# QData/ChromeGCN

Hardware: AMD Instinct MI355X
Metric: GCN windows/sec (2-layer, d_model=128) on GM12878 Hi-C graph (higher is better)
Workload: dtype f32

## Files before the change

chromegcn_amd/csrc/cgcn_common.hpp:

```cpp
#pragma once
#include <hip/hip_runtime.h>
#include <stdint.h>

#include "chromegcn.h"

typedef float f32x4 __attribute__((ext_vector_type(4)));
typedef float f32x2 __attribute__((ext_vector_type(2)));

#define WAVE 64
#define TILE_NODES 16
#ifndef BWD_MAX_PARTIALS
#define BWD_MAX_PARTIALS 256
#endif

typedef __bf16 bf16x8 __attribute__((ext_vector_type(8)));
typedef __bf16 bf16x2 __attribute__((ext_vector_type(2)));
typedef uint32_t u32x4 __attribute__((ext_vector_type(4)));
typedef uint32_t u32x2 __attribute__((ext_vector_type(2)));
__device__ __forceinline__ uint32_t sp_pack(float x0, float x1) {
  return __builtin_bit_cast(uint32_t, __builtin_convertvector((f32x2){x0, x1}, bf16x2));
}
__device__ __forceinline__ float sp_lo(uint32_t pk) { return __uint_as_float(pk << 16); }
__device__ __forceinline__ float sp_up(uint32_t pk) { return __uint_as_float(pk & 0xffff0000u); }
__device__ __forceinline__ void sp_split2(float x0, float x1, uint32_t& h, uint32_t& m, uint32_t& l) {
// ... 182 lines not shown
__device__ __forceinline__ void bacc_add(unsigned long long* b, int S, int D, int slot, int s, int c, double sdy, double sdyx,
                                         int fa, int fb) {
  unsigned long long* w = b + ((size_t)(slot * S + s) * D + c) * 2;
  const double va = ldexp(sdy, fa), vb = ldexp(sdyx, fb);
  if (!(__builtin_fabs(va) < 1.15e18) || !(__builtin_fabs(vb) < 1.15e18)) {
    atomicOr(b + (size_t)STAT_ACC_SLOTS * S * D * 2 + BACC_FLAG, 1ull);
    atomicOr(b + (size_t)STAT_ACC_SLOTS * S * D * 2 + BACC_LOSS, BACC_LOSS_BAD);
    return;
  }
  atomicAdd(&w[0], (unsigned long long)(long long)__builtin_rint(va));
  atomicAdd(&w[1], (unsigned long long)(long long)__builtin_rint(vb));
}
__device__ __forceinline__ void bacc_get(const unsigned long long* __restrict__ b, int S, int D, int s, int c, int n, float& c0, float& c1) {
  long long ta = 0, tb = 0;
#pragma unroll
  for (int slot = 0; slot < STAT_ACC_SLOTS; ++slot) {
    const unsigned long long* w = b + ((size_t)(slot * S + s) * D + c) * 2;
    ta += (long long)w[0];
    tb += (long long)w[1];
  }
  const unsigned long long* h = b + (size_t)STAT_ACC_SLOTS * S * D * 2;
  const int fa = (int)(unsigned)(h[BACC_EXP] & 0xFFFFFFFFull) - 1024, fb = (int)(unsigned)(h[BACC_EXP] >> 32) - 1024;
  const double invn = 1.0 / (double)n;
  c0 = (float)(ldexp((double)ta, -fa) * invn);
  c1 = (float)(ldexp((double)tb, -fb) * invn);
  if (h[BACC_FLAG] != 0ull) c0 = c1 = __builtin_nanf("");
}
__device__ __forceinline__ void stat_acc_add(unsigned long long* acc, int S, int D, int slot, int s, int c, double sum1, double sum2,
                                             double lim = 4194304.0) {
  const double sc = (double)(1ll << STAT_ACC_FBITS);
  unsigned long long* w = acc + ((size_t)(slot * S + s) * D + c) * 2;
  if (!(__builtin_fabs(sum1) < lim) || !(sum2 < lim)) {
    atomicOr(acc + (size_t)STAT_ACC_SLOTS * S * D * 2, 1ull);
    return;
  }
  atomicAdd(&w[0], (unsigned long long)(long long)__builtin_rint(sum1 * sc));
  atomicAdd(&w[1], (unsigned long long)(long long)__builtin_rint(sum2 * sc));
}
__device__ __forceinline__ void stat_acc_get(const unsigned long long* __restrict__ acc, int S, int D, int s, int c, int n,
                                             double& mean, double& m2) {
  long long t1 = 0, t2 = 0;
#pragma unroll
  for (int slot = 0; slot < STAT_ACC_SLOTS; ++slot) {
    const unsigned long long* w = acc + ((size_t)(slot * S + s) * D + c) * 2;
    t1 += (long long)w[0];
    t2 += (long long)w[1];
  }
  const double isc = 1.0 / (double)(1ll << STAT_ACC_FBITS);
  const double s1 = (double)t1 * isc, s2 = (double)t2 * isc;
  mean = s1 / (double)n;
  m2 = s2 - mean * s1;
  if (m2 < 0.0) m2 = 0.0;
  if (acc[(size_t)STAT_ACC_SLOTS * S * D * 2] != 0ull) mean = m2 = __builtin_nan("");
}

#define HEAD_STREAM_ID 0x4845u

struct HeadApply {
  const float* dym;
  const float* bnc;
  const unsigned long long* bacc;
  const float* mean;
  const float* invstd;
  const float* bn_w;
  const unsigned long long* rng_state;
  float keep_scale;
  uint32_t thresh;
  int S;
  const float* hf_part;
  float* hf_dWout;
  float* hf_dbout;
  int hf_P, hf_C, hf_CP, hf_accumulate;
  const float* dloss;
  float* hf_dbn_w;
  float* hf_dbn_b;
};

__host__ __device__ __forceinline__ constexpr int head_part_stride(int CP, int D) { return CP * D + CP + 8 * D; }
#define HEAD_STAT_COLS 16

template <int NT, bool EXT = false>
__device__ __forceinline__ void head_finalize_slab(int slab, int P, int D, int C, int CP,
                                                   const float* __restrict__ part, float* __restrict__ dWout,
                                                   float* __restrict__ dbout, int accumulate,
                                                   const float* __restrict__ dloss, void* scratch = nullptr) {
  constexpr int NS = NT / 64;
  const float gl = dloss ? dloss[0] : 1.f;
  const int PS = head_part_stride(CP, D);
  const int total = CP * D + CP;
  float (*hred)[64];
  if constexpr (EXT) {
    hred = (float (*)[64])scratch;
  } else {
    __shared__ __attribute__((aligned(16))) float hred_own[NS][64];
    hred = hred_own;
  }
  const int lane = threadIdx.x & 63, wave = threadIdx.x >> 6;
  const int el4 = lane & 15, sub = lane >> 4;
  const int e0 = slab * 64 + el4 * 4;
  f32x4 a = {0.f, 0.f, 0.f, 0.f};
  if (e0 < total) {
    const int per = (P + NS * 4 - 1) / (NS * 4);
    const int p0 = (wave * 4 + sub) * per, p1 = min(P, p0 + per);
    for (int p = p0; p < p1; p += 8) {
      f32x4 t[8];
#pragma unroll
// ... 117 lines not shown
```

chromegcn_amd/csrc/cgcn_head.hip:

```cpp
#include "cgcn_common.hpp"

#define HEAD_STAT_BLOCKS 128
#define HEAD_TILE 16
#define HEADB_TILE 32
#ifndef HEAD_MAX_PARTIALS
#define HEAD_MAX_PARTIALS 256
#endif


template <int D>
__global__ __launch_bounds__(256) void k_head_colstats(int n, int S, int rows_per_blk, const float* __restrict__ X,
                                                       float* __restrict__ part) {
  constexpr int RL = 256 / D;
  __shared__ float sm[2][256];
  const int c = threadIdx.x % D, rl = threadIdx.x / D;
  const int r0 = blockIdx.x * rows_per_blk, r1 = min(n, r0 + rows_per_blk);
  for (int s = 0; s < S; ++s) {
    const float* Xs = X + (size_t)s * n * D + c;
    const float pivot = r0 < n ? fmaxf(Xs[(size_t)r0 * D], 0.f) : 0.f;
    float s1 = 0.f, s2 = 0.f;
    int i = r0 + rl;
    for (; i + 3 * RL < r1; i += 4 * RL) {
      float v[4];
#pragma unroll
// ... 976 lines not shown
      for (int e = 0; e < EPL; ++e) {
        const int c = lane * EPL + e;
        const float g = gv[e];
#pragma unroll
        for (int s = 0; s < 2; ++s) {
          if (s < S) {
            float dy = g * invS;
            if (thresh) dy = dropout_keep(key, (uint32_t)(((size_t)s * n + i) * D + c), thresh) ? dy * keep_scale : 0.f;
            const float xh = (fmaxf(xv[t][s][e], 0.f) - mu[s][e]) * is[s][e];
            sdy[s][e] += dy;
            sdyx[s][e] += dy * xh;
          }
        }
      }
    }
    __syncthreads();
  }

  HF_STAMP(10);
  float* P = part + (size_t)blockIdx.x * PS;
#pragma unroll
  for (int ib = 0; ib < CBMAX; ++ib)
#pragma unroll
    for (int jb = 0; jb < JBW; ++jb)
#pragma unroll
      for (int e = 0; e < 4; ++e)
        if (c0 + ib * 16 < CPT) P[(size_t)(c0 + ib * 16 + q * 4 + e) * D + (wave * JBW + jb) * 16 + r] = accW[ib][jb][e];
  if (threadIdx.x < CP && c0 + (int)threadIdx.x < CPT) P[CPT * D + c0 + threadIdx.x] = dbo;
  HF_STAMP(11);
  lacc = wave_sum(lacc);
  if (lane == 0) lsum[wave] = lacc;
  if (last) {
    unsigned long long* bb = sa.acc ? bacc_base(sa.acc, S, D) : nullptr;
    int fa = 0, fb = 0;
    if (sa.acc) {
      head_bacc_points(wmax, NW, keep_scale, n, fa, fb);
      if (blockIdx.x == 0 && threadIdx.x == 0)
        bb[(size_t)STAT_ACC_SLOTS * S * D * 2 + BACC_EXP] = ((unsigned long long)(unsigned)(fb + 1024) << 32) | (unsigned long long)(unsigned)(fa + 1024);
    }
    head_stats_partial<D, NW, TR * LDY>(Yt, (double*)(P + CPT * D + CPT), sdy, sdyx, wave, lane, bb, S, fa, fb);
  }
  __syncthreads();
  if (threadIdx.x == 0) {
    float t = 0.f;
#pragma unroll
    for (int w = 0; w < NW; ++w) t += lsum[w];
    const float tl = first ? t : loss_part[blockIdx.x] + t;
    loss_part[blockIdx.x] = tl;
    if (sa.acc && last) head_loss_ticket(sa, S, D, tl, inv_count);
  }
  HF_STAMP(12);
}

#if (defined(HRSX_NOBACC) || defined(HRSX_NOSTAGE) || defined(HRSX_NOTICKET)) && !defined(CGCN_EXPERIMENT_BUILD)
#error "HRSX_* are decomposition switches (garbage results): build a variant with -DCGCN_EXPERIMENT_BUILD (tools/mkvariant.py), never the shipped library"
#endif
#ifndef HEAD_RS
#define HEAD_RS 1
#endif
#ifndef HEAD_NT_PROBS
#define HEAD_NT_PROBS 0
#endif
#ifndef HEAD_RS_PRIO
#define HEAD_RS_PRIO 0
#endif
#ifdef RS_TIMING
__device__ unsigned long long rs_stamps[8 * 2 * 8];
#ifndef RS_STAMP_K
#define RS_STAMP_K 1
#endif
#define RS_STAMP(i)                                                                                        \
  do {                                                                                                     \
    __builtin_amdgcn_s_waitcnt(0);                                                                         \
    if (k == RS_STAMP_K && (threadIdx.x == 0 || threadIdx.x == 512) && (blockIdx.x & 31) == 0)             \
      rs_stamps[((blockIdx.x >> 5) * 2 + (threadIdx.x >> 9)) * 8 + (i)] = wall_clock64();                  \
  } while (0)
extern "C" int cgcn_debug_rs_stamps(unsigned long long* out) {
  return hipMemcpyFromSymbol(out, HIP_SYMBOL(rs_stamps), sizeof(unsigned long long) * 8 * 2 * 8) == hipSuccess ? 0 : -1;
}
#else
#define RS_STAMP(i)
#endif
template <bool MULTI, int NB, bool DROP, int NRB = 2>
__global__ __launch_bounds__(1024) void k_head_fused_rs(int n, int S, int C, const float* __restrict__ X,
                                                        const float* __restrict__ bn_w, const float* __restrict__ bn_b,
                                                        const float* __restrict__ mean, const float* __restrict__ invstd,
                                                        const float* __restrict__ Wout, const float* __restrict__ bout,
                                                        const float* __restrict__ target, float keep_scale, uint32_t thresh,
                                                        const unsigned long long* __restrict__ rng_state, float inv_count,
                                                        float* __restrict__ probs, float* __restrict__ loss_part,
                                                        float* __restrict__ dym, float* __restrict__ part,
                                                        int c0, int Cp, int CPT, int first_, int last_, HeadStatAcc sa) {
  constexpr int D = 128, TR = 16 * NRB, EPL = 2, RPW = TR / 8, KQ = D / 4;
  constexpr int CP = 128, CBMAX = 8;
  constexpr int LDP = CP + 18, LDY = D + 16, LDW = D + 16;
  __shared__ __attribute__((aligned(16))) float Wl[NB * 16 * LDW];
  __shared__ __attribute__((aligned(16))) float Pt[2][TR * LDP];
  __shared__ __attribute__((aligned(16))) float Yt[2][TR * LDY];
  __shared__ float lsum[8];
  __shared__ float wmax[16];
  const bool first = MULTI ? first_ != 0 : true, last = MULTI ? last_ != 0 : true;

  const int lane = threadIdx.x & 63;
  const int wave = __builtin_amdgcn_readfirstlane(threadIdx.x >> 6);
  const int own = wave & 7;
  const uint32_t key = DROP ? dropout_key(rng_state, HEAD_STREAM_ID) : 0u;
  const float invS = 1.f / (float)S;
// ... 642 lines not shown
        const int c = own * 16 + r;
#pragma unroll
        for (int e = 0; e < 4; ++e) {
          const int i = node0 + q * 4 + e;
          const float g = accY[e];
          if (i < n) dym[(unsigned)(i * D + c)] = g;
          if (last) {
#pragma unroll
            for (int s = 0; s < 2; ++s) {
              float dy = g * invS;
              if (DROP) dy = dropout_keep(key, (uint32_t)((s * n + i) * D + c), thresh) ? dy * keep_scale : 0.f;
              if (s == 1) dy = S2 ? dy : 0.f;
              const float xh = (fmaxf(xq[s][e], 0.f) - mu[s]) * is[s];
              sdy[s] += dy;
              sdyx[s] += dy * xh;
            }
          }
        }
      }
      __syncthreads();
      if (k < mt) load_xq((int)blockIdx.x + k * G);
      if (k >= 1) {
        int lq = lane;
        asm volatile("" : "+v"(lq));
        const int hh = lq >> 5, c16 = (lq >> 4) & 1, qp = (lq & 15) >> 2, pp = lq & 3;
        const int cbk = own >> 1, lb0 = 2 * (own & 1);
        const unsigned char* __restrict__ Pb = Ptb[(k - 1) & 1];
        const unsigned char* __restrict__ Yb = Ytb[(k - 1) & 1];
        int ty[2], tp[2];
#pragma unroll
        for (int rd = 0; rd < 2; ++rd) {
          const int row = 8 * hh + 4 * rd + qp, sg = sp_sigma(row);
          ty[rd] = row * 256 + (((4 * cbk + 2 * c16 + (pp >> 1)) ^ sg) << 4) + ((pp & 1) << 3);
          tp[rd] = row * 256 + (((4 * lb0 + 2 * c16 + (pp >> 1)) ^ sg) << 4) + ((pp & 1) << 3);
        }
        bf16x8 yf[3];
#pragma unroll
        for (int v = 0; v < 3; ++v) yf[v] = tr_pair(Yb + v * LVT + ty[0], Yb + v * LVT + ty[1]);
#pragma unroll
        for (int bb = 0; bb < 2; ++bb) {
          bf16x8 pf[3];
#pragma unroll
          for (int v = 0; v < 3; ++v) pf[v] = tr_pair(Pb + v * LVT + (tp[0] ^ (bb << 6)), Pb + v * LVT + (tp[1] ^ (bb << 6)));
          accW[bb] = __builtin_amdgcn_mfma_f32_32x32x16_bf16(pf[2], yf[0], accW[bb], 0, 0, 0);
          accW[bb] = __builtin_amdgcn_mfma_f32_32x32x16_bf16(pf[0], yf[2], accW[bb], 0, 0, 0);
          accW[bb] = __builtin_amdgcn_mfma_f32_32x32x16_bf16(pf[1], yf[1], accW[bb], 0, 0, 0);
          accW[bb] = __builtin_amdgcn_mfma_f32_32x32x16_bf16(pf[1], yf[0], accW[bb], 0, 0, 0);
          accW[bb] = __builtin_amdgcn_mfma_f32_32x32x16_bf16(pf[0], yf[1], accW[bb], 0, 0, 0);
          accW[bb] = __builtin_amdgcn_mfma_f32_32x32x16_bf16(pf[0], yf[0], accW[bb], 0, 0, 0);
        }
      }
      __syncthreads();
    }
    {
      const int hh = lane >> 5, cbk = own >> 1, lb0 = 2 * (own & 1);
#pragma unroll
      for (int bb = 0; bb < 2; ++bb)
#pragma unroll
        for (int e = 0; e < 16; ++e) {
          const int lab = 32 * (lb0 + bb) + (e & 3) + 8 * (e >> 2) + 4 * hh;
          if (c0 + (lab & ~15) < CPT) P[(size_t)(c0 + lab) * D + 32 * cbk + (lane & 31)] = accW[bb][e];
        }
    }
    const int r = lane & 15, q = lane >> 4;
    if (last) {
      double* out = (double*)(P + CPT * D + CPT);
#pragma unroll
      for (int s = 0; s < 2; ++s) {
        double a = (double)sdy[s], b = (double)sdyx[s];
        a += __shfl_xor(a, 16); a += __shfl_xor(a, 32);
        b += __shfl_xor(b, 16); b += __shfl_xor(b, 32);
        if (q == 0) {
          out[s * D + own * 16 + r] = a;
          out[(2 + s) * D + own * 16 + r] = b;
          if (sa.acc && s < S) {
            int fa, fb;
            head_bacc_points(wmax, 16, keep_scale, n, fa, fb);
            unsigned long long* bb = bacc_base(sa.acc, S, D);
#ifndef HRSX_NOBACC
            bacc_add(bb, S, D, (int)blockIdx.x & (STAT_ACC_SLOTS - 1), s, own * 16 + r, a, b, fa, fb);
#endif
            if (blockIdx.x == 0 && s == 0 && own == 0 && r == 0)
              bb[(size_t)STAT_ACC_SLOTS * S * D * 2 + BACC_EXP] = ((unsigned long long)(unsigned)(fb + 1024) << 32) | (unsigned long long)(unsigned)(fa + 1024);
          }
        }
      }
    }
    __syncthreads();
  }
#undef OPAQUE_LANE
}

__global__ __launch_bounds__(512) void k_head_bwd_finalize(int wslab0, int wslabs, int P, int n, int S, int D, int C, int CP,
                                                           const float* __restrict__ part, float* __restrict__ dWout,
                                                           float* __restrict__ dbout, float* __restrict__ dbn_w,
                                                           float* __restrict__ dbn_b, float* __restrict__ bnc,
                                                           int accumulate, const float* __restrict__ dloss) {
  if ((int)blockIdx.x < wslabs)
    head_finalize_slab<512>(wslab0 + blockIdx.x, P, D, C, CP, part, dWout, dbout, accumulate, dloss);
  else
    head_stats_finalize<512>((int)blockIdx.x - wslabs, P, n, S, D, CP, part, dbn_w, dbn_b, bnc, accumulate, dloss);
}

__global__ __launch_bounds__(512) void k_head_train_finish(int P, int n, int S, int D, int CP,
                                                           const float* __restrict__ part, float* __restrict__ bnc,
                                                           const float* __restrict__ loss_part, float inv_count,
// ... 360 lines not shown
```

chromegcn_amd/csrc/cgcn_kernels.hip:

```cpp
#include <atomic>
#include <type_traits>
#include <cstdlib>

#include "cgcn_common.hpp"

template <int S, int D>
struct Geo {
  static constexpr int PAY = S * D;
  static constexpr bool HALF = (PAY == 128);
  static constexpr int NV = HALF ? 1 : PAY / 256;
  static_assert(PAY == 128 || PAY == 256 || PAY == 512, "unsupported payload");
  __device__ static __forceinline__ int strand(int v, int lane) { return HALF ? 0 : ((v * 64 + lane) * 4) / D; }
  __device__ static __forceinline__ int column(int v, int lane) { return HALF ? (lane & 31) * 4 : ((v * 64 + lane) * 4) % D; }
};

#ifndef GU_OVERRIDE
#define GU_OVERRIDE 0
#endif
#ifndef NT_SAVED
#define NT_SAVED 0
#endif
#if NT_SAVED
#define NT_STORE4(p, v) __builtin_nontemporal_store((v), (f32x4*)(p))
#define NT_STORE1(p, v) __builtin_nontemporal_store((v), (p))
// ... 956 lines not shown
#pragma unroll
        for (int rr = 0; rr < R; ++rr) {
          v[rr] = St[(s * R + rr) * LD + c];
          sum += rr < cnt ? v[rr] : 0.f;
        }
        const float mean = sum * inv;
        float m2 = 0.f;
#pragma unroll
        for (int rr = 0; rr < R; ++rr) m2 += rr < cnt ? (v[rr] - mean) * (v[rr] - mean) : 0.f;
        chan_combine(st_cnt, st_mean, st_m2, (float)cnt, mean, m2);
      }
    }
  }
  if (colstats && threadIdx.x < S * D && tfirst < tend) {
    if (stat_acc) {
      const double nb = (double)st_cnt, mb = (double)st_mean;
      stat_acc_add((unsigned long long*)colstats, S, D, (int)blockIdx.x & (STAT_ACC_SLOTS - 1), (int)threadIdx.x / D,
                   (int)threadIdx.x % D, nb * mb, (double)st_m2 + nb * mb * mb);
    } else {
      float* out = colstats + ((size_t)blockIdx.x * S * D + threadIdx.x) * 2;
      out[0] = st_mean;
      out[1] = st_m2;
    }
  }
}

#ifndef RING_SLOTS
#define RING_SLOTS 8
#endif
#ifndef RING_ROW_WAVES
#define RING_ROW_WAVES 8
#endif
#define RING_THREADS ((RING_ROW_WAVES + 8) * 64)
#ifndef RING_PF
#define RING_PF 2
#endif
#ifndef RING_PF_HEAD
#define RING_PF_HEAD 2
#endif
#ifndef RING_PRIO
#define RING_PRIO 1
#endif
#ifndef RING_OPBUF
#define RING_OPBUF 2
#endif
#ifndef RING_EARLY_FLAG
#define RING_EARLY_FLAG 1
#endif
#ifndef RING_PRIME
#define RING_PRIME 0
#endif
#if (defined(RING_NO_WAIT) || defined(RING_SKIP_MFMA) || defined(RING_SKIP_ROWTEAM) || defined(RING_SKIP_LOADS) || \
     defined(RING_TEST_SLOW_ROW) || defined(RING_TEST_SLOW_MATRIX) || defined(RL256_SKIP_MFMA) || defined(RL256_SKIP_LOADS) || \
     defined(BSX_NORIDERS) || defined(BSX_NODXN) || defined(BSX_NOSTORE)) && \
    !defined(CGCN_EXPERIMENT_BUILD)
#error "RING_NO_WAIT / RING_SKIP_* / RING_TEST_SLOW_* are experiment switches: build a variant with -DCGCN_EXPERIMENT_BUILD (tools/mkvariant.py), never the shipped library"
#endif
#if defined(RING_TEST_SLOW_ROW) || defined(RING_TEST_SLOW_MATRIX)
__device__ __forceinline__ void ring_test_delay(int wave, int it) {
  unsigned h = (unsigned)wave * 2654435761u ^ (unsigned)it * 40503u ^ (unsigned)blockIdx.x * 97u;
  h ^= h >> 7;
  for (unsigned i = 0; i < (h & 15u); ++i) __builtin_amdgcn_s_sleep(10);
}
#endif
__device__ __forceinline__ void ring_wait(const unsigned* flag, unsigned target) {
#ifdef RING_NO_WAIT
  return;
#endif
  unsigned long long t0 = 0;
  for (unsigned spins = 1;; ++spins) {
    const unsigned v = __builtin_amdgcn_readfirstlane(__hip_atomic_load(flag, __ATOMIC_RELAXED, __HIP_MEMORY_SCOPE_WORKGROUP));
    if ((int)(v - target) >= 0) break;
    if ((spins & 0xFFFFu) == 0u) {
      const unsigned long long now = __builtin_amdgcn_s_memrealtime();
      if (t0 == 0) t0 = now;
      else if (now - t0 > 1000000000ull) __builtin_trap();
    }
    __builtin_amdgcn_s_sleep(1);
  }
  asm volatile("" ::: "memory");
}
__device__ __forceinline__ void ring_arrive(unsigned* flag, int lane) {
  asm volatile("s_waitcnt lgkmcnt(0)" ::: "memory");
  if (lane == 0) __hip_atomic_fetch_add(flag, 1u, __ATOMIC_RELAXED, __HIP_MEMORY_SCOPE_WORKGROUP);
}
#ifndef RING_SLOTS_SP
#define RING_SLOTS_SP 6
#endif
template <bool HEAD, bool DROP, int PROD>
__global__ __launch_bounds__(RING_THREADS) void k_bwd_rowlocal_ring(int M, int n, const float* __restrict__ dXn,
                                                            const float* __restrict__ Z, const float* __restrict__ X,
                                                            const float* __restrict__ gate, const float* __restrict__ dgate,
                                                            const float* __restrict__ H, const float* __restrict__ wg,
                                                            const float* __restrict__ rs, float* __restrict__ dHs,
                                                            float* __restrict__ part, HeadApply hp,
                                                            float* __restrict__ dxn_store, int row_blocks, int head_slabs,
                                                            const float* __restrict__ W) {
  constexpr int D = 128, SR = 16, NSL = PROD ? RING_SLOTS_SP : RING_SLOTS, PF = HEAD ? RING_PF_HEAD : RING_PF;
  constexpr int SLOT_F = PROD ? 3 * SR * D / 2 : SR * D;
  constexpr int LVB = SR * D * 2;
  constexpr int NRW = RING_ROW_WAVES;
  constexpr int NT = RING_THREADS;
  constexpr int RT = SR / (2 * NRW);
  static_assert(NRW * 2 * RT == SR && (NRW == 4 || NRW == 8), "row-team geometry");
  constexpr int PSTRIDE = D * D + 2 * D + 4;
  constexpr int RS = 2 * D + 4;
  __shared__ __attribute__((aligned(16))) float Hs[NSL][SLOT_F];
// ... 176 lines not shown
          unsigned char* hb = (unsigned char*)Hs[slot] + wo;
          *(u32x2*)hb = h2;
          *(u32x2*)(hb + LVB) = m2;
          *(u32x2*)(hb + 2 * LVB) = l2;
          sp_split4(du[t], h2, m2, l2);
          unsigned char* ub = (unsigned char*)Us[slot] + wo;
          *(u32x2*)ub = h2;
          *(u32x2*)(ub + LVB) = m2;
          *(u32x2*)(ub + 2 * LVB) = l2;
        } else {
          *(f32x4*)&Hs[slot][rowi * D + ((l ^ ((rowi & 1) << 2)) << 2)] = w.h[t];
          *(f32x4*)&Us[slot][rowi * D + ((l ^ rowi) << 2)] = du[t];
        }
        if (l == 0) Sc[slot][rowi] = w.sc[t];
      }
#endif
      ring_arrive(&FULL[slot], lane);
    };
#ifdef RING_SKIP_ROWTEAM
    __syncthreads();
    for (int it = 0; it < ns; ++it) {
      if (it >= NSL) ring_wait(&FREE[it % NSL], 8u * (unsigned)(it / NSL));
      ring_arrive(&FULL[it % NSL], lane);
    }
#else
#pragma unroll
    for (int j = 0; j < PF; ++j)
      if (j < ns) load_slot(j, R_[j]);
    __syncthreads();
    for (int it0 = 0; it0 < ns; it0 += PF) {
#pragma unroll
      for (int j = 0; j < PF; ++j) {
        const int it = it0 + j;
        if (it < ns) {
          row_pass(it, R_[j]);
          if (it + PF < ns) load_slot(it + PF, R_[j]);
        }
      }
    }
#endif
#pragma unroll
    for (int e = 0; e < 4; ++e) {
      db_acc[e] += __shfl_xor(db_acc[e], 32);
      dwg_acc[e] += __shfl_xor(dwg_acc[e], 32);
    }
    dcg_acc += __shfl_xor(dcg_acc, 32);
    if (!upper) {
      *(f32x4*)&red[wave][4 * l] = db_acc;
      *(f32x4*)&red[wave][D + 4 * l] = dwg_acc;
      if (l == 0) red[wave][2 * D] = dcg_acc;
    }
    ring_arrive(DONE, lane);
    ring_wait(DONE, (unsigned)NRW);
    for (int c = threadIdx.x; c < 2 * D + 1; c += NRW * 64) {
      float sacc = 0.f;
#pragma unroll
      for (int w = 0; w < NRW; ++w) sacc += red[w][c];
      P[D * D + c] = sacc;
    }
  } else if constexpr (PROD != 0) {
    const int own = wave - NRW;
    int lq = lane;
    asm volatile("" : "+v"(lq));
    const int r16 = lq & 15, q4 = lq >> 4;
    bf16x8 th[4], tm[4], tl[4];
#pragma unroll
    for (int s4 = 0; s4 < 4; ++s4) {
      float v[8];
      const f32x4 v0 = dHs ? *(const f32x4*)&W[(size_t)(16 * own + r16) * D + 32 * s4 + 8 * q4] : (f32x4){0.f, 0.f, 0.f, 0.f};
      const f32x4 v1 = dHs ? *(const f32x4*)&W[(size_t)(16 * own + r16) * D + 32 * s4 + 8 * q4 + 4] : (f32x4){0.f, 0.f, 0.f, 0.f};
#pragma unroll
      for (int u = 0; u < 4; ++u) {
        v[u] = v0[u];
        v[4 + u] = v1[u];
      }
      sp_split8(v, th[s4], tm[s4], tl[s4]);
    }
    f32x16 accW[2];
#pragma unroll
    for (int bb = 0; bb < 2; ++bb)
#pragma unroll
      for (int e = 0; e < 16; ++e) accW[bb][e] = 0.f;
    __syncthreads();
    if (RING_PRIO) __builtin_amdgcn_s_setprio(RING_PRIO);
    const int hh = lq >> 5, c16 = (lq >> 4) & 1, qp = (lq & 15) >> 2, pp = lq & 3;
    const int hcb = own >> 1, ucb = own & 1;
    int trH[2], trU[2];
#pragma unroll
    for (int rd = 0; rd < 2; ++rd) {
      const int row = 8 * hh + 4 * rd + qp, sg = sp_sigma(row);
      trH[rd] = row * 256 + (((4 * hcb + 2 * c16 + (pp >> 1)) ^ sg) << 4) + ((pp & 1) << 3);
      trU[rd] = row * 256 + (((8 * ucb + 2 * c16 + (pp >> 1)) ^ sg) << 4) + ((pp & 1) << 3);
    }
    const int ua0 = r16 * 256 + ((q4 ^ (sp_sigma(r16) & 3)) << 4), ua_hi = sp_sigma(r16) >> 2;
    const unsigned dh_lane = (unsigned)(4 * q4 * D + own * 16 + r16);
    bool next_full = false;
    auto slot_loop = [&](auto DH_) {
      constexpr bool DH = decltype(DH_)::value;
      for (int it = 0; it < ns; ++it) {
        const int slot = it % NSL;
#ifdef RING_TEST_SLOW_MATRIX
        ring_test_delay(wave, it);
#endif
#ifndef RING_SKIP_MFMA
        const unsigned char* Hb = (const unsigned char*)Hs[slot];
        const unsigned char* Ub = (const unsigned char*)Us[slot];
        if (!(RING_EARLY_FLAG && next_full)) ring_wait(&FULL[slot], (unsigned)NRW * (unsigned)(it / NSL + 1));
        bf16x8 hf[3], uf[3];
#pragma unroll
        for (int v = 0; v < 3; ++v) hf[v] = tr_pair(Hb + v * LVB + trH[0], Hb + v * LVB + trH[1]);
        SpAcc2 sa;
        sa.zero();
#pragma unroll
        for (int bb = 0; bb < 2; ++bb) {
#pragma unroll
          for (int v = 0; v < 3; ++v) uf[v] = tr_pair(Ub + v * LVB + (trU[0] ^ (bb << 6)), Ub + v * LVB + (trU[1] ^ (bb << 6)));
          accW[bb] = __builtin_amdgcn_mfma_f32_32x32x16_bf16(hf[2], uf[0], accW[bb], 0, 0, 0);
          accW[bb] = __builtin_amdgcn_mfma_f32_32x32x16_bf16(hf[0], uf[2], accW[bb], 0, 0, 0);
          accW[bb] = __builtin_amdgcn_mfma_f32_32x32x16_bf16(hf[1], uf[1], accW[bb], 0, 0, 0);
          accW[bb] = __builtin_amdgcn_mfma_f32_32x32x16_bf16(hf[1], uf[0], accW[bb], 0, 0, 0);
          accW[bb] = __builtin_amdgcn_mfma_f32_32x32x16_bf16(hf[0], uf[1], accW[bb], 0, 0, 0);
          accW[bb] = __builtin_amdgcn_mfma_f32_32x32x16_bf16(hf[0], uf[0], accW[bb], 0, 0, 0);
          if (DH) {
#pragma unroll
            for (int s2 = 0; s2 < 2; ++s2) {
              const int s4 = 2 * bb + s2;
              const int o = ua0 + ((s4 ^ ua_hi) << 6);
              const bf16x8 ah = __builtin_bit_cast(bf16x8, *(const u32x4*)(Ub + o));
              const bf16x8 am = __builtin_bit_cast(bf16x8, *(const u32x4*)(Ub + LVB + o));
              const bf16x8 al = __builtin_bit_cast(bf16x8, *(const u32x4*)(Ub + 2 * LVB + o));
              sa.step(ah, am, al, th[s4], tm[s4], tl[s4]);
            }
          }
        }
        f32x4 sc_cur = {0.f, 0.f, 0.f, 0.f};
        if (DH) sc_cur = *(const f32x4*)&Sc[slot][4 * q4];
        if (RING_EARLY_FLAG) {
          const unsigned nflag = __hip_atomic_load(&FULL[(it + 1) % NSL], __ATOMIC_RELAXED, __HIP_MEMORY_SCOPE_WORKGROUP);
          next_full = it + 1 < ns && (int)(__builtin_amdgcn_readfirstlane(nflag) - (unsigned)NRW * (unsigned)((it + 1) / NSL + 1)) >= 0;
          asm volatile("" ::: "memory");
        }
        ring_arrive(&FREE[slot], lane);
        if (DH) {
          const f32x4 hacc = sa.sum();
          const int m0 = (s_begin + it) * SR + 4 * q4;
          const unsigned o = (unsigned)((s_begin + it) * SR * D) + dh_lane;
          if ((s_begin + it) * SR + SR <= M) {
#pragma unroll
            for (int e = 0; e < 4; ++e) dHs[o + e * D] = hacc[e] * sc_cur[e];
          } else {
#pragma unroll
            for (int e = 0; e < 4; ++e)
              if (m0 + e < M) dHs[o + e * D] = hacc[e] * sc_cur[e];
          }
        }
#else
        ring_wait(&FULL[slot], (unsigned)NRW * (unsigned)(it / NSL + 1));
        ring_arrive(&FREE[slot], lane);
#endif
      }
    };
    if (dHs) slot_loop(std::true_type{});
    else slot_loop(std::false_type{});
#pragma unroll
    for (int bb = 0; bb < 2; ++bb)
#pragma unroll
      for (int e = 0; e < 16; ++e)
        P[(32 * hcb + (e & 3) + 8 * (e >> 2) + 4 * hh) * D + 64 * ucb + 32 * bb + (lq & 31)] = accW[bb][e];
  } else {
    const int own = wave - NRW;
    int lq = lane;
    asm volatile("" : "+v"(lq));
    const int r = lq & 15, q = lq >> 4;
    f32x4 accW[8], WT[8];
#pragma unroll
    for (int i = 0; i < 8; ++i) accW[i] = (f32x4){0.f, 0.f, 0.f, 0.f};
#pragma unroll
    for (int t = 0; t < 8; ++t) WT[t] = dHs ? *(const f32x4*)&W[(size_t)(16 * own + r) * D + 16 * t + 4 * q] : (f32x4){0.f, 0.f, 0.f, 0.f};
    __syncthreads();
    if (RING_PRIO) __builtin_amdgcn_s_setprio(RING_PRIO);
    const int ha_off = q * D + (((4 * own + (r >> 2)) ^ ((q & 1) << 2)) << 2) + (r & 3);
    const int ub_lo = q * D + (((r & 3) ^ q) << 2);
    const int ua_lo = r * D + ((q ^ (r & 3)) << 2);
    const int rq = r >> 2;
    const unsigned dh_lane = (unsigned)(4 * q * D + own * 16 + r);
    constexpr int OB = RING_OPBUF;
    float av[4];
    f32x4 bv[OB], uv[OB];
    bool primed = false, next_full = false;
    auto slot_loop = [&](auto DH_) {
      constexpr bool DH = decltype(DH_)::value;
      auto rd = [&](const float* __restrict__ Hb, const float* __restrict__ Ub, int s) {
        const int kk = s >> 1, h = s & 1;
        if (h == 0) av[kk] = Hb[ha_off + kk * 4 * D];
        bv[s % OB] = *(const f32x4*)&Ub[ub_lo + kk * 4 * D + 64 * h + ((rq ^ kk) << 4)];
        if (DH) uv[s % OB] = *(const f32x4*)&Ub[ua_lo + (((s & 3) ^ rq) << 4) + (s & 4) * 16];
      };
      for (int it = 0; it < ns; ++it) {
        const int slot = it % NSL;
#ifdef RING_TEST_SLOW_MATRIX
        ring_test_delay(wave, it);
#endif
#ifndef RING_SKIP_MFMA
        const float* __restrict__ Hb = Hs[slot];
        const float* __restrict__ Ub = Us[slot];
        if (!primed) {
          if (!(RING_EARLY_FLAG && next_full)) ring_wait(&FULL[slot], (unsigned)NRW * (unsigned)(it / NSL + 1));
          rd(Hb, Ub, 0);
        }
        if (OB == 3) rd(Hb, Ub, 1);
        f32x4 sc_cur;
        primed = false;
        const int nslot = (it + 1) % NSL;
        unsigned nflag = 0u;
        f32x4 hacc = {0.f, 0.f, 0.f, 0.f};
#pragma unroll
        for (int s = 0; s < 8; ++s) {
          if (s + OB - 1 < 8) rd(Hb, Ub, s + OB - 1);
          if (s == 5 && (RING_PRIME || RING_EARLY_FLAG)) nflag = __hip_atomic_load(&FULL[nslot], __ATOMIC_RELAXED, __HIP_MEMORY_SCOPE_WORKGROUP);
          if (DH && s == 7) sc_cur = *(const f32x4*)&Sc[slot][4 * q];
          if (s == 7 && RING_EARLY_FLAG) {
            next_full = it + 1 < ns &&
                        (int)(__builtin_amdgcn_readfirstlane(nflag) - (unsigned)NRW * (unsigned)((it + 1) / NSL + 1)) >= 0;
            asm volatile("" ::: "memory");
          }
          if (s == 7 && RING_PRIME && it + 1 < ns &&
              (int)(__builtin_amdgcn_readfirstlane(nflag) - (unsigned)NRW * (unsigned)((it + 1) / NSL + 1)) >= 0) {
            asm volatile("" ::: "memory");
            primed = true;
            rd(Hs[nslot], Us[nslot], 0);
          }
          __builtin_amdgcn_sched_barrier(0);
          const int kk = s >> 1, h = s & 1;
#pragma unroll
          for (int u = 0; u < 4; ++u) {
            accW[h * 4 + u] = __builtin_amdgcn_mfma_f32_16x16x4f32(av[kk], bv[s % OB][u], accW[h * 4 + u], 0, 0, 0);
            if (DH) {
              hacc = __builtin_amdgcn_mfma_f32_16x16x4f32(uv[s % OB][u], WT[s][u], hacc, 0, 0, 0);
              if (u < 3) __builtin_amdgcn_sched_barrier(0);
            }
          }
          __builtin_amdgcn_sched_barrier(0);
        }
        ring_arrive(&FREE[slot], lane);
        if (DH) {
          const int m0 = (s_begin + it) * SR + 4 * q;
          const unsigned o = (unsigned)((s_begin + it) * SR * D) + dh_lane;
          if ((s_begin + it) * SR + SR <= M) {
#pragma unroll
            for (int e = 0; e < 4; ++e) dHs[o + e * D] = hacc[e] * sc_cur[e];
          } else {
#pragma unroll
            for (int e = 0; e < 4; ++e)
              if (m0 + e < M) dHs[o + e * D] = hacc[e] * sc_cur[e];
          }
        }
#else
        ring_wait(&FULL[slot], (unsigned)NRW * (unsigned)(it / NSL + 1));
        ring_arrive(&FREE[slot], lane);
#endif
      }
    };
    if (dHs) slot_loop(std::true_type{});
    else slot_loop(std::false_type{});
#pragma unroll
    for (int h = 0; h < 2; ++h)
#pragma unroll
      for (int e = 0; e < 4; ++e)
        *(f32x4*)&P[(own * 16 + q * 4 + e) * D + 64 * h + 4 * r] = (f32x4){accW[h * 4 + 0][e], accW[h * 4 + 1][e], accW[h * 4 + 2][e], accW[h * 4 + 3][e]};
  }
}

#ifndef RL256_ROW_WAVES
#define RL256_ROW_WAVES 8
#endif
#define RL256_THREADS ((RL256_ROW_WAVES + 8) * 64)
#ifndef RL256_PRIO
#define RL256_PRIO 1
#endif
#ifndef RL256_ROW_PRIO
#define RL256_ROW_PRIO 0
#endif
template <int TR>
__global__ __launch_bounds__(RL256_THREADS) void k_bwd_rowlocal256s(int M, int n, const float* __restrict__ dXn,
                                                          const float* __restrict__ Z, const float* __restrict__ X,
                                                          const float* __restrict__ gate, const float* __restrict__ dgate,
                                                          const float* __restrict__ H, const float* __restrict__ wg,
                                                          const float* __restrict__ rs, float* __restrict__ dHs,
                                                          float* __restrict__ part, HeadApply hp,
                                                          float* __restrict__ dxn_store, int row_blocks, int head_slabs,
                                                          const float* __restrict__ W) {
  constexpr int D = 256, NRW = RL256_ROW_WAVES, NT = RL256_THREADS, SW = 64;
  static_assert(TR == 32, "one 16 x 16 dHs tile per matrix wave needs 32-row tiles");
  constexpr int LD = D + 16, EPL = D / 64, RPW = TR / NRW, PSTRIDE = D * D + 2 * D + 4, RS = 2 * D + 4;
  static_assert(EPL == 4, "one 16-byte chunk per lane");
  __shared__ __attribute__((aligned(16))) float Hs[2][TR * LD];
  if ((int)blockIdx.x >= row_blocks) {
    const int extra = (int)blockIdx.x - row_blocks;
    const int wslabs = (hp.hf_CP * D + hp.hf_CP) / 64;
    static_assert(sizeof(Hs) >= 4 * (NT / HEAD_STAT_COLS) * (HEAD_STAT_COLS + 1) * sizeof(double), "finalize staging fits the H slots");
    if (extra < wslabs)
      head_finalize_slab<NT, true>(extra, hp.hf_P, D, hp.hf_C, hp.hf_CP, hp.hf_part, hp.hf_dWout, hp.hf_dbout,
                                   hp.hf_accumulate, hp.dloss, &Hs[0][0]);
    else
      head_stats_finalize<NT, true>(extra - wslabs, hp.hf_P, n, hp.S, D, hp.hf_CP, hp.hf_part, hp.hf_dbn_w, hp.hf_dbn_b,
                                    nullptr, hp.hf_accumulate, hp.dloss, &Hs[0][0]);
    return;
  }
  __shared__ __attribute__((aligned(16))) float Us[2][TR * LD];
  __shared__ __attribute__((aligned(16))) float red[NRW][RS];
  __shared__ unsigned flg[5];
  __shared__ float Hc[2 * 2 * D];
  const int lane = threadIdx.x & 63;
  const int wave = __builtin_amdgcn_readfirstlane(threadIdx.x >> 6);
  if (hp.dym && hp.bacc) {
    for (int idx = threadIdx.x; idx < hp.S * D; idx += NT) {
      const int s = idx / D, c = idx % D;
      float c0, c1;
      bacc_get(bacc_base(hp.bacc, hp.S, D), hp.S, D, s, c, n, c0, c1);
      Hc[(s * 2 + 0) * D + c] = c0;
      Hc[(s * 2 + 1) * D + c] = c1;
    }
// ... 74 lines not shown
            ld_row<EPL>(bw_, &hp.bn_w[lane * EPL]);
            if (hp.bacc) {
              ld_row<EPL>(c0, &Hc[(s * 2 + 0) * D + lane * EPL]);
              ld_row<EPL>(c1, &Hc[(s * 2 + 1) * D + lane * EPL]);
            } else {
              ld_row<EPL>(c0, &hp.bnc[(s * 2 + 0) * D + lane * EPL]);
              ld_row<EPL>(c1, &hp.bnc[(s * 2 + 1) * D + lane * EPL]);
            }
#pragma unroll
            for (int e = 0; e < EPL; ++e) {
              const float xn = (1.f - g) * x[t][e] + g * z[t][e];
              float dy = gup[t][e] * invS * hgl;
              if (hp.thresh) dy = dropout_keep(hkey, (uint32_t)(off + e), hp.thresh) ? dy * hp.keep_scale : 0.f;
              const float xh = (fmaxf(xn, 0.f) - mu[e]) * is[e];
              const float dr = bw_[e] * is[e] * (dy - hgl * c0[e] - xh * (hgl * c1[e]));
              gup[t][e] = xn > 0.f ? dr : 0.f;
            }
            if (dxn_store && cs == 0) st_row<EPL>(&dxn_store[off], gup[t]);
          }
          float dg = 0.f;
#pragma unroll
          for (int e = 0; e < EPL; ++e) dg += gup[t][e] * (z[t][e] - x[t][e]);
          dg = wave_sum(dg) + dgt[t];
          const float gamma = g * (1.f - g) * dg;
#pragma unroll
          for (int e = 0; e < EPL; ++e) {
            const float dz = g * gup[t][e] + gamma * wgl[e];
            du[e] = dz * (1.f - z[t][e] * z[t][e]);
            db_acc[e] += du[e];
            dwg_acc[e] += gamma * z[t][e];
          }
          dcg_acc += gamma;
        } else {
#pragma unroll
          for (int e = 0; e < EPL; ++e) du[e] = 0.f;
        }
        *(f32x4*)&Ht[trow * LD + lane * EPL] = (f32x4){h[t][0], h[t][1], h[t][2], h[t][3]};
        *(f32x4*)&Ut[trow * LD + lane * EPL] = (f32x4){du[0], du[1], du[2], du[3]};
        if (tt + RIF < RPW) load_row(it, tt + RIF);
        else load_row(it + 1, tt + RIF - RPW);
      }
      ring_arrive(&FULL[slot], lane);
      KT_STAMP_NW(2 + 2 * it, 0, it < 3);
    }
    KT_STAMP_NW(7, 0, true);
#pragma unroll
    for (int e = 0; e < EPL; ++e) {
      red[wave][lane * EPL + e] = db_acc[e];
      red[wave][D + lane * EPL + e] = dwg_acc[e];
    }
    if (lane == 0) red[wave][2 * D] = dcg_acc;
    ring_arrive(DONE, lane);
    ring_wait(DONE, (unsigned)NRW);
    for (int c = threadIdx.x; c < 2 * D + 1; c += NRW * 64) {
      const int col = c < D ? c : (c < 2 * D ? c - D : -1);
      const bool mine = col >= 0 ? (col >= SW * cs && col < SW * cs + SW) : (cs == 0);
      if (!mine) continue;
      float sacc = 0.f;
#pragma unroll
      for (int w = 0; w < NRW; ++w) sacc += red[w][c];
      P[D * D + c] = sacc;
    }
  } else {
    const int own = wave - NRW;
    const int r = lane & 15, q = lane >> 4;
    const int rb = own >> 2, cb = own & 3;
    f32x4 R[2][4];
#pragma unroll
    for (int ib = 0; ib < 2; ++ib)
#pragma unroll
      for (int jb = 0; jb < 4; ++jb) R[ib][jb] = (f32x4){0.f, 0.f, 0.f, 0.f};
    f32x4 WT[16];
#pragma unroll
    for (int t = 0; t < 16; ++t)
      WT[t] = dHs ? *(const f32x4*)&W[(size_t)(SW * cs + 16 * cb + r) * D + 16 * t + 4 * q] : (f32x4){0.f, 0.f, 0.f, 0.f};
    __syncthreads();
    if (RL256_PRIO) __builtin_amdgcn_s_setprio(RL256_PRIO);
    auto tile_loop = [&](auto DH_) {
      constexpr bool DH = decltype(DH_)::value;
      for (int it = 0; it < nt; ++it) {
        const int slot = it & 1;
        const float* __restrict__ Ht = Hs[slot];
        const float* __restrict__ Ut = Us[slot];
        KT_STAMP_NW(8, NRW * 64, it == 0);
        ring_wait(&FULL[slot], (unsigned)NRW * (unsigned)((it >> 1) + 1));
        KT_STAMP_NW(9 + 2 * it, NRW * 64, it < 3);
        f32x4 hacc = {0.f, 0.f, 0.f, 0.f};
#ifndef RL256_SKIP_MFMA
#pragma unroll
        for (int kk = 0; kk < TR / 4; ++kk) {
          const int k = 4 * kk + q;
          float a[2], bq[4];
#pragma unroll
          for (int ib = 0; ib < 2; ++ib) a[ib] = Ht[k * LD + (2 * own + ib) * 16 + r];
#pragma unroll
          for (int jb = 0; jb < 4; ++jb) bq[jb] = Ut[k * LD + SW * cs + jb * 16 + r];
          f32x4 ua[2];
          if (DH) {
            ua[0] = *(const f32x4*)&Ut[(16 * rb + r) * LD + 16 * (2 * kk) + 4 * q];
            ua[1] = *(const f32x4*)&Ut[(16 * rb + r) * LD + 16 * (2 * kk + 1) + 4 * q];
          }
#pragma unroll
          for (int jb = 0; jb < 4; ++jb)
#pragma unroll
            for (int ib = 0; ib < 2; ++ib) {
              R[ib][jb] = __builtin_amdgcn_mfma_f32_16x16x4f32(a[ib], bq[jb], R[ib][jb], 0, 0, 0);
// ... 39 lines not shown
__device__ __forceinline__ void sgd_apply(const SgdFuse& sg, int idx, float g) {
  const float pi = sg.param[idx];
  const float d = g * sg.grad_scale + sg.wd * pi;
  float upd = d;
  if (sg.mom) {
    const float b = sg.mu * sg.mom[idx] + d;
    sg.mom[idx] = b;
    upd = sg.nesterov ? d + sg.mu * b : b;
  }
  sg.param[idx] = pi - sg.lr * upd;
}

template <int NT>
__device__ __forceinline__ void reduce_slab(int slab, int P, int D, const float* __restrict__ part,
                                            float* __restrict__ dW, float* __restrict__ db, float* __restrict__ dwg,
                                            float* __restrict__ dcg, int accumulate, const SgdFuse& sg) {
  constexpr int NS = NT / 64;
  const int PSTRIDE = D * D + 2 * D + 4;
  const int total = D * D + 2 * D + 1;
  __shared__ __attribute__((aligned(16))) float red[NS][64];
  const int lane = threadIdx.x & 63, wave = threadIdx.x >> 6;
  const int el4 = lane & 15, sub = lane >> 4;
  const int e0 = slab * 64 + el4 * 4;
  f32x4 a = {0.f, 0.f, 0.f, 0.f};
  if (e0 < total) {
    const int per = (P + NS * 4 - 1) / (NS * 4);
    const int p0 = (wave * 4 + sub) * per, p1 = min(P, p0 + per);
    for (int p = p0; p < p1; p += 8) {
      f32x4 t[8];
#pragma unroll
      for (int u = 0; u < 8; ++u) t[u] = *(const f32x4*)(part + (size_t)min(p + u, p1 - 1) * PSTRIDE + e0);
#pragma unroll
      for (int u = 0; u < 8; ++u)
        if (p + u < p1) a += t[u];
    }
  }
#pragma unroll
  for (int k = 0; k < 4; ++k) {
    float v = a[k];
    v += __shfl_xor(v, 16);
    v += __shfl_xor(v, 32);
    a[k] = v;
  }
  if (sub == 0) *(f32x4*)&red[wave][el4 * 4] = a;
  const int el = threadIdx.x & 63, slice = threadIdx.x >> 6;
  const int e = slab * 64 + el;
  float s;
  __syncthreads();
  if (slice == 0 && e < total) {
    s = 0.f;
#pragma unroll
    for (int w = 0; w < NS; ++w) s += red[w][el];
    float* dst;
    if (e < D * D) dst = dW + e;
    else if (e < D * D + D) dst = db + (e - D * D);
    else if (e < D * D + 2 * D) dst = dwg + (e - D * D - D);
    else dst = dcg;
    *dst = accumulate ? (*dst + s) : s;
    if (sg.param) sgd_apply(sg, (int)(dst - sg.grad), s);
  }
}

#ifndef REDUCE_WIDE_MAX_P
#define REDUCE_WIDE_MAX_P 64
#endif
template <int NT>
__device__ __forceinline__ void reduce_slab_wide(int wg, int P, int D, const float* __restrict__ part,
                                                 float* __restrict__ dW, float* __restrict__ db, float* __restrict__ dwg,
                                                 float* __restrict__ dcg, int accumulate, const SgdFuse& sg) {
  constexpr int NW = NT / 64;
  const int PSTRIDE = D * D + 2 * D + 4;
  const int total = D * D + 2 * D + 1;
  __shared__ __attribute__((aligned(16))) float redw[NW][256];
  const int lane = threadIdx.x & 63, wave = threadIdx.x >> 6;
  const int e0 = wg * 256 + lane * 4;
  f32x4 a = {0.f, 0.f, 0.f, 0.f};
  if (e0 < PSTRIDE) {
    const int per = (P + NW - 1) / NW;
    const int p0 = wave * per, p1 = min(P, p0 + per);
    for (int p = p0; p < p1; p += 8) {
      f32x4 t[8];
#pragma unroll
      for (int u = 0; u < 8; ++u) t[u] = *(const f32x4*)(part + (size_t)min(p + u, p1 - 1) * PSTRIDE + e0);
#pragma unroll
      for (int u = 0; u < 8; ++u)
        if (p + u < p1) a += t[u];
    }
  }
  *(f32x4*)&redw[wave][lane * 4] = a;
  __syncthreads();
  const int e = wg * 256 + (int)threadIdx.x;
  if (threadIdx.x < 256 && e < total) {
    float s = 0.f;
#pragma unroll
    for (int w = 0; w < NW; ++w) s += redw[w][threadIdx.x];
    float* dst;
    if (e < D * D) dst = dW + e;
    else if (e < D * D + D) dst = db + (e - D * D);
    else if (e < D * D + 2 * D) dst = dwg + (e - D * D - D);
    else dst = dcg;
    *dst = accumulate ? (*dst + s) : s;
    if (sg.param) sgd_apply(sg, (int)(dst - sg.grad), s);
  }
}

__device__ __forceinline__ void sgd_other_elements(const SgdFuse& sg, int block, int D, const float* dW, const float* db,
                                                   const float* dwg, const float* dcg) {
  const int i = block * (int)blockDim.x + (int)threadIdx.x;
  if (i == 0 && sg.rng_state) sg.rng_state[1] += 1ull;
  if (i < sg.count) {
    const float* gp = sg.grad + i;
    const bool mine = (gp >= dW && gp < dW + D * D) || (gp >= db && gp < db + D) || (gp >= dwg && gp < dwg + D) || gp == dcg;
    if (!mine) sgd_apply(sg, i, *gp);
  }
}

__global__ __launch_bounds__(256) void k_reduce_partials(int P, int D, const float* __restrict__ part,
                                                         float* __restrict__ dW, float* __restrict__ db,
                                                         float* __restrict__ dwg, float* __restrict__ dcg,
                                                         int accumulate, SgdFuse sg, int reduce_slabs) {
  if ((int)blockIdx.x >= reduce_slabs) {
    sgd_other_elements(sg, (int)blockIdx.x - reduce_slabs, D, dW, db, dwg, dcg);
    return;
  }
  reduce_slab<256>(blockIdx.x, P, D, part, dW, db, dwg, dcg, accumulate, sg);
}

#ifndef SLICED_HUB
#define SLICED_HUB 192
#endif
#ifndef SLICED_COST_MODEL
#define SLICED_COST_MODEL 1
#endif
#ifndef SLICED_COOP_OVERHEAD
#define SLICED_COOP_OVERHEAD 3
#endif
template <int U>
__device__ __forceinline__ int group8_bcast(int v) { return __builtin_amdgcn_ds_swizzle(v, 0x18 | (U << 5)); }

template <int U, bool HAS_VAL>
struct SlicedBcast {
  static __device__ __forceinline__ void run(unsigned (&off)[8], float (&w)[8], int myc, float myv, unsigned rowsh,
                                             unsigned lane_off) {
    SlicedBcast<U - 1, HAS_VAL>::run(off, w, myc, myv, rowsh, lane_off);
    off[U - 1] = ((unsigned)group8_bcast<U - 1>(myc) << rowsh) + lane_off;
    if (HAS_VAL) w[U - 1] = __int_as_float(group8_bcast<U - 1>(__float_as_int(myv)));
  }
};
template <bool HAS_VAL>
struct SlicedBcast<0, HAS_VAL> {
// ... 1124 lines not shown
```

Before: 58.65 million.

## Store weight-gradient partials in MFMA-native record layout and remap in reduction

```diff
diff --git a/chromegcn_amd/csrc/cgcn_common.hpp b/chromegcn_amd/csrc/cgcn_common.hpp
--- a/chromegcn_amd/csrc/cgcn_common.hpp
+++ b/chromegcn_amd/csrc/cgcn_common.hpp
@@ -258,6 +258,22 @@
   m2 = s2 - mean * s1;
   if (m2 < 0.0) m2 = 0.0;
   if (acc[(size_t)STAT_ACC_SLOTS * S * D * 2] != 0ull) mean = m2 = __builtin_nan("");
+}
+
+__host__ __device__ __forceinline__ constexpr int rec128_index(int row, int col) {
+  return (((row >> 5) * 4 + (col >> 5)) << 10) + (((row >> 3) & 3) << 8) + ((((row >> 2) & 1) * 32 + (col & 31)) << 2) + (row & 3);
+}
+__host__ __device__ __forceinline__ constexpr int rec128_elem(int idx) {
+  return (32 * (idx >> 12) + 8 * ((idx >> 8) & 3) + 4 * ((idx >> 7) & 1) + (idx & 3)) * 128 + 32 * ((idx >> 10) & 3) + ((idx >> 2) & 31);
+}
+static_assert(rec128_elem(rec128_index(77, 101)) == 77 * 128 + 101 && rec128_index(127, 127) == 128 * 128 - 1, "rec128_index / rec128_elem");
+
+#ifndef REC_STORE_AUX
+#define REC_STORE_AUX 16
+#endif
+__device__ __forceinline__ void store16_wt(float* base, unsigned byte_off, f32x4 v, unsigned bytes) {
+  const __amdgpu_buffer_rsrc_t r = __builtin_amdgcn_make_buffer_rsrc(base, 0, (int)bytes, 0x00020000);
+  __builtin_amdgcn_raw_buffer_store_b128(__builtin_bit_cast(u32x4, v), r, (int)byte_off, 0, REC_STORE_AUX);
 }
 
 #define HEAD_STREAM_ID 0x4845u
diff --git a/chromegcn_amd/csrc/cgcn_head.hip b/chromegcn_amd/csrc/cgcn_head.hip
--- a/chromegcn_amd/csrc/cgcn_head.hip
+++ b/chromegcn_amd/csrc/cgcn_head.hip
@@ -1052,7 +1052,7 @@
   HF_STAMP(12);
 }
 
-#if (defined(HRSX_NOBACC) || defined(HRSX_NOSTAGE) || defined(HRSX_NOTICKET)) && !defined(CGCN_EXPERIMENT_BUILD)
+#if (defined(HRSX_NOBACC) || defined(HRSX_NOSTAGE) || defined(HRSX_NOTICKET) || defined(HRSX_NORECORDS)) && !defined(CGCN_EXPERIMENT_BUILD)
 #error "HRSX_* are decomposition switches (garbage results): build a variant with -DCGCN_EXPERIMENT_BUILD (tools/mkvariant.py), never the shipped library"
 #endif
 #ifndef HEAD_RS
@@ -1801,6 +1801,9 @@
       }
       __syncthreads();
     }
+#ifdef HRSX_NORECORDS
+    if (n < 0)
+#endif
     {
       const int hh = lane >> 5, cbk = own >> 1, lb0 = 2 * (own & 1);
 #pragma unroll
diff --git a/chromegcn_amd/csrc/cgcn_kernels.hip b/chromegcn_amd/csrc/cgcn_kernels.hip
--- a/chromegcn_amd/csrc/cgcn_kernels.hip
+++ b/chromegcn_amd/csrc/cgcn_kernels.hip
@@ -1032,7 +1032,7 @@
 #endif
 #if (defined(RING_NO_WAIT) || defined(RING_SKIP_MFMA) || defined(RING_SKIP_ROWTEAM) || defined(RING_SKIP_LOADS) || \
      defined(RING_TEST_SLOW_ROW) || defined(RING_TEST_SLOW_MATRIX) || defined(RL256_SKIP_MFMA) || defined(RL256_SKIP_LOADS) || \
-     defined(BSX_NORIDERS) || defined(BSX_NODXN) || defined(BSX_NOSTORE)) && \
+     defined(BSX_NORIDERS) || defined(BSX_NODXN) || defined(BSX_NOSTORE) || defined(RING_NORECORDS)) && \
     !defined(CGCN_EXPERIMENT_BUILD)
 #error "RING_NO_WAIT / RING_SKIP_* / RING_TEST_SLOW_* are experiment switches: build a variant with -DCGCN_EXPERIMENT_BUILD (tools/mkvariant.py), never the shipped library"
 #endif
@@ -1315,11 +1315,18 @@
     }
     ring_arrive(DONE, lane);
     ring_wait(DONE, (unsigned)NRW);
-    for (int c = threadIdx.x; c < 2 * D + 1; c += NRW * 64) {
-      float sacc = 0.f;
-#pragma unroll
-      for (int w = 0; w < NRW; ++w) sacc += red[w][c];
-      P[D * D + c] = sacc;
+#ifdef RING_NORECORDS
+    if (M < 0)
+#endif
+    for (int c = threadIdx.x; 2 * c < RS; c += NRW * 64) {
+      f32x2 sacc = {0.f, 0.f};
+#pragma unroll
+      for (int w = 0; w < NRW; ++w) {
+        if (2 * c < 2 * D + 1) sacc[0] += red[w][2 * c];
+        if (2 * c + 1 < 2 * D + 1) sacc[1] += red[w][2 * c + 1];
+      }
+      __hip_atomic_store((unsigned long long*)&P[D * D + 2 * c], __builtin_bit_cast(unsigned long long, sacc), __ATOMIC_RELAXED,
+                         __HIP_MEMORY_SCOPE_AGENT);
     }
   } else if constexpr (PROD != 0) {
     const int own = wave - NRW;
@@ -1425,11 +1432,15 @@
     };
     if (dHs) slot_loop(std::true_type{});
     else slot_loop(std::false_type{});
+#ifdef RING_NORECORDS
+    if (M < 0)
+#endif
 #pragma unroll
     for (int bb = 0; bb < 2; ++bb)
 #pragma unroll
-      for (int e = 0; e < 16; ++e)
-        P[(32 * hcb + (e & 3) + 8 * (e >> 2) + 4 * hh) * D + 64 * ucb + 32 * bb + (lq & 31)] = accW[bb][e];
+      for (int g = 0; g < 4; ++g)
+        store16_wt(P, 4u * (unsigned)(((4 * hcb + 2 * ucb + bb) << 10) + (g << 8) + (lq << 2)),
+                   (f32x4){accW[bb][4 * g], accW[bb][4 * g + 1], accW[bb][4 * g + 2], accW[bb][4 * g + 3]}, D * D * 4);
   } else {
     const int own = wave - NRW;
     int lq = lane;
@@ -1529,8 +1540,7 @@
 #pragma unroll
     for (int h = 0; h < 2; ++h)
 #pragma unroll
-      for (int e = 0; e < 4; ++e)
-        *(f32x4*)&P[(own * 16 + q * 4 + e) * D + 64 * h + 4 * r] = (f32x4){accW[h * 4 + 0][e], accW[h * 4 + 1][e], accW[h * 4 + 2][e], accW[h * 4 + 3][e]};
+      for (int u = 0; u < 4; ++u) *(f32x4*)&P[rec128_index(own * 16 + q * 4, 64 * h + 4 * r + u)] = accW[h * 4 + u];
   }
 }
 
@@ -1711,6 +1721,9 @@
     if (lane == 0) red[wave][2 * D] = dcg_acc;
     ring_arrive(DONE, lane);
     ring_wait(DONE, (unsigned)NRW);
+#ifdef RING_NORECORDS
+    if (M < 0)
+#endif
     for (int c = threadIdx.x; c < 2 * D + 1; c += NRW * 64) {
       const int col = c < D ? c : (c < 2 * D ? c - D : -1);
       const bool mine = col >= 0 ? (col >= SW * cs && col < SW * cs + SW) : (cs == 0);
@@ -1856,7 +1869,7 @@
 #pragma unroll
     for (int w = 0; w < NS; ++w) s += red[w][el];
     float* dst;
-    if (e < D * D) dst = dW + e;
+    if (e < D * D) dst = dW + (D == 128 ? rec128_elem(e) : e);
     else if (e < D * D + D) dst = db + (e - D * D);
     else if (e < D * D + 2 * D) dst = dwg + (e - D * D - D);
     else dst = dcg;
@@ -1899,7 +1912,7 @@
 #pragma unroll
     for (int w = 0; w < NW; ++w) s += redw[w][threadIdx.x];
     float* dst;
-    if (e < D * D) dst = dW + e;
+    if (e < D * D) dst = dW + (D == 128 ? rec128_elem(e) : e);
     else if (e < D * D + D) dst = db + (e - D * D);
     else if (e < D * D + 2 * D) dst = dwg + (e - D * D - D);
     else dst = dcg;
```

After: 58.21 million. About the same (-0.8%).
